# Ladme/groan_rs

Measured on AMD Instinct MI355X. Metric: frames/sec RMSD-fit, 1e6 atoms triclinic, 1/2/4/8 GPUs; HBM GB/s vs peak, higher is better.
Workload: dtype f32 (fp64 accumulators)

## Files before the change

groan_rs_amd/csrc/gr_api.hip:

```cpp
#include <hip/hip_runtime.h>

#include <cmath>
#include <cstdio>
#include <cstdlib>
#include <cstring>
#include <map>
#include <string>
#include <vector>

#include "../../include/groan_hip.h"
#include "gr_container.h"
#include "gr_kernels.h"
#include "gr_hot.h"
#include "gr_resident.h"
#include "gr_small.h"
#include "gr_xtc.h"
#include "gr_shape.h"
#include "gr_xtc_dev.h"
#include "gr_xtc_enc_dev.h"
#include "gr_trr.h"
#include "gr_cellgrid.h"
#include "gr_textio.h"
#include "gr_pool.h"
#include <set>
// ... 71 lines not shown
    int stream_wgs_cu = 0;
    int translate_rows = 1;
    int center_resident = 1;
    uint64_t cen_res_launches = 0, cen_res_redone = 0;
    int res_fit_last = 0;
    struct Metro { uint64_t shape = 0; double free_ns = 0, T_ns = 0, best_ns = 0, fail_ns = 0; uint32_t off_for = 0, held = 0; } metro;
    uint64_t res_metro_period_ns = 0, res_last_turn_ns = 0, res_late_permille = 0, res_sclk_mhz = 0;
    int wall_khz = 100000;
    uint32_t res_max_wgs = 0;
    int res_test_no_start = 0;
    uint32_t res_test_abort_at = 0xFFFFFFFFu;
    uint32_t res_skip = 0, res_backoff = 0;
    uint32_t *res_progress = nullptr;
    unsigned long long *res_wgrec = nullptr; size_t res_wgrec_cap = 0;
    unsigned long long *res_rec = nullptr;
    uint32_t *res_abort = nullptr;
    uint32_t *res_words_host = nullptr;
    struct ResOut { GrFrameState st[GR_MAX_BATCH]; uint32_t words[16]; alignas(64) uint32_t seq; };
    ResOut *res_out = nullptr, *res_out_dev = nullptr;
    uint32_t res_seq = 0;
    uint32_t res_checkin = 0, res_closed = 0;
    uint32_t res_late_seen[2] = { 0, 0 };
    uint64_t res_lean_segments = 0, res_sync_fallbacks = 0;
    GrShapeSet *shape_set_dev = nullptr;
    unsigned long long *shape_mask_dev = nullptr, *shape_mask_host = nullptr; size_t shape_mask_cap = 0;
    uint32_t res_epoch = 0;
    bool res_in_use = false;
    uint64_t res_launches = 0, res_handshake_misses = 0, res_aborts = 0, res_redone_frames = 0;
    GrFrameState *state_dev = nullptr;
    GrFrameState *state_host = nullptr;
    GrFrameState *small_state = nullptr, *small_state_dev = nullptr;
    uint32_t *small_flag = nullptr, *small_flag_dev = nullptr;
    uint32_t small_seq = 0;
    uint32_t small_max = GR_SMALL_MAX_DEFAULT;
    uint64_t small_calls = 0, small_sync_fallbacks = 0;
    uint32_t *bad_dev = nullptr;
// ... 388 lines not shown
            HIPCHK(c, hipStreamSynchronize(c->stream));
            if (w[0] != seq || w[words - 1] != seq) return fail(c, GR_E_HIP, "a single-wave kernel ended without publishing its result");
            break;
        }
    }
    std::atomic_thread_fence(std::memory_order_acquire);
    c->small_calls++;
    return GR_OK;
}

static int res_next_epoch(gr_ctx *c, uint32_t *epoch) {
    if (++c->res_epoch == 0u) {
        HIPCHK(c, hipStreamSynchronize(c->stream));
        if (c->res_wgrec) HIPCHK(c, hipMemset(c->res_wgrec, 0, c->res_wgrec_cap * sizeof(unsigned long long)));
        HIPCHK(c, hipMemset(c->res_rec, 0, (size_t)GR_MAX_BATCH * 16 * sizeof(unsigned long long)));
        HIPCHK(c, hipMemset(c->res_abort + 2, 0, 2 * sizeof(uint32_t)));
        c->res_epoch = 1u;
    }
    *epoch = c->res_epoch;
    return GR_OK;
}
static int res_test_no_start(gr_ctx *c, uint32_t epoch) {
    if (!c->res_test_no_start) return GR_OK;
    const unsigned long long two = 2ull | ((unsigned long long)epoch << 32);
    c->res_test_no_start = 0;
    HIPCHK(c, hipMemcpyAsync(c->res_abort + 2, &two, sizeof two, hipMemcpyHostToDevice, c->stream));
    HIPCHK(c, hipStreamSynchronize(c->stream));
    return GR_OK;
}
template <int MODE>
static int res_close(gr_ctx *c, uint32_t nb, const double *fit_partials, uint32_t nparts, double sum_w, uint32_t epoch, bool fresh, uint32_t *seq) {
    const uint32_t sq = c->res_seq + 1u;
    k_res_close<MODE><<<dim3(nb), dim3(64), 0, c->stream>>>(fit_partials, nparts, sum_w, c->state_dev, c->res_rec, epoch, fresh ? 1u : 0u, c->res_abort, c->res_closed + nb,
                                                        c->res_out_dev->st, c->res_out_dev->words, &c->res_out_dev->seq, sq);
    HIPCHK(c, hipGetLastError());
    c->res_seq = sq; c->res_closed += nb; *seq = sq;
    return GR_OK;
}
static int res_collect(gr_ctx *c, uint32_t seq, uint32_t nb, uint32_t epoch, bool *started) {
    volatile uint32_t *w = &c->res_out->seq;
    const auto t0 = std::chrono::steady_clock::now();
    for (uint32_t spins = 0; *w != seq; ++spins) {
        if ((spins & 1023u) == 1023u && std::chrono::steady_clock::now() - t0 > std::chrono::milliseconds(20)) {
            c->res_sync_fallbacks++;
            HIPCHK(c, hipStreamSynchronize(c->stream));
            if (*w != seq) return fail(c, GR_E_HIP, "the kernel behind the resident pass ended without publishing its results");
            break;
        }
    }
    std::atomic_thread_fence(std::memory_order_acquire);
    memcpy(c->state_host, c->res_out->st, (size_t)nb * sizeof(GrFrameState));
    memcpy(c->res_words_host, c->res_out->words, 12 * sizeof(uint32_t));
    for (int k = 0; k < 2; ++k) { const uint32_t v = c->res_words_host[8 + k]; c->res_words_host[8 + k] = v - c->res_late_seen[k]; c->res_late_seen[k] = v; }
    *started = c->res_words_host[2] == 1u && c->res_words_host[3] == epoch;
    if (!*started || c->res_words_host[0]) HIPCHK(c, hipStreamSynchronize(c->stream));
    return GR_OK;
}

int center_stage(gr_ctx *c, uint32_t first_slot, uint32_t nf, const GrSel &sel, int kind, int weighted,
                 int mass_first, int target, int only_status = 0) {
    if (small_ok(c, sel)) {
// ... 189 lines not shown
    (void)hipSetDevice(c->device);
    if (c->copy_stream) (void)hipStreamSynchronize(c->copy_stream);
    if (c->stream) (void)hipStreamSynchronize(c->stream);
    resident_done(c);
    whole_release(c);
    for (auto &kv : c->groups) { if (kv.second.idx_dev) (void)hipFree(kv.second.idx_dev); if (kv.second.mask_dev) (void)hipFree(kv.second.mask_dev); }
    if (c->frames) (void)hipFree(c->frames);
    if (c->aos_up) (void)hipFree(c->aos_up);
    if (c->aos_dl) (void)hipFree(c->aos_dl);
    if (c->masses) (void)hipFree(c->masses);
    if (c->boxes_dev) (void)hipFree(c->boxes_dev);
    if (c->boxes_host) (void)hipHostFree(c->boxes_host);
    if (c->cen_partials) (void)hipFree(c->cen_partials);
    if (c->acc_partials) (void)hipFree(c->acc_partials);
    if (c->fit_partials) (void)hipFree(c->fit_partials);
    if (c->fuse_cnt) (void)hipFree(c->fuse_cnt);
    if (c->res_abort) (void)hipFree(c->res_abort);
    if (c->res_words_host) (void)hipHostFree(c->res_words_host);
    if (c->res_out) (void)hipHostFree(c->res_out);
    if (c->shape_set_dev) (void)hipFree(c->shape_set_dev);
    if (c->shape_mask_dev) (void)hipFree(c->shape_mask_dev);
    if (c->shape_mask_host) (void)hipHostFree(c->shape_mask_host);
    if (c->res_wgrec) (void)hipFree(c->res_wgrec);
    if (c->res_rec) (void)hipFree(c->res_rec);
    if (c->res_progress) (void)hipFree(c->res_progress);
    if (c->state_dev) (void)hipFree(c->state_dev);
    if (c->state_host) (void)hipHostFree(c->state_host);
    if (c->small_state) (void)hipHostFree(c->small_state);
    if (c->bad_dev) (void)hipFree(c->bad_dev);
    if (c->bad_host) (void)hipHostFree(c->bad_host);
// ... 875 lines not shown
    }
    GrResCtl ctl;
    memset(&ctl, 0, sizeof ctl);
    { const int se = res_next_epoch(c, &ctl.epoch); if (se) return se; }
    ctl.wgrec = c->res_wgrec; ctl.rec = c->res_rec; ctl.abort = c->res_abort; ctl.progress = c->res_progress; ctl.n_stream = res_stream; ctl.n_fin = n_fin;
    ctl.checkin_target = c->res_checkin + res_stream + n_fin; ctl.fresh_states = fresh_states ? 1u : 0u;
    ctl.wgs_frame = wgs; ctl.streams = streams; ctl.groups_wg = gwg;
    ctl.team_waves = resident_team_waves(wgs, streams);
    ctl.patience_ticks = (unsigned long long)c->wall_khz * 3000ull; ctl.start_ticks = (unsigned long long)c->wall_khz * 200ull;
    ctl.test_abort_frame = c->res_test_abort_at; c->res_test_abort_at = 0xFFFFFFFFu;
    ctl.metro_t16 = c->res_metro_ns >= 100 ? (uint32_t)std::min<uint64_t>(0xFFFFFFFFull, (uint64_t)c->res_metro_ns * (uint64_t)c->wall_khz * 16ull / 1000000ull) : 0u;
    ctl.metro_lead = (uint32_t)((uint64_t)c->wall_khz * 2000ull / 1000000ull);
    ctl.cen_weighted = weighted ? 1u : 0u; ctl.cen_dim_mask = (uint32_t)dim_mask;
    float *frames = c->frames; size_t stride = c->frame_stride; uint32_t slot0 = s0, nfr = nb, natoms = (uint32_t)c->n;
    const float *masses = c->masses; GrSel sel_arg = csel; const GrBox *boxes = c->boxes_dev; GrPlanDev plan; memset(&plan, 0, sizeof plan);
    GrFrameState *states = c->state_dev; double *fparts = nullptr;
    void *args[] = { &frames, &stride, &slot0, &nfr, &natoms, &masses, &sel_arg, &boxes, &plan, &states, &fparts, &ctl };
    bool ubox = true;
    for (uint32_t f = 1; f < nb && ubox; ++f) ubox = memcmp(&c->boxes_host[s0 + f], &c->boxes_host[s0], sizeof(GrBox)) == 0;
    const bool fit_last = c->res_fit_last ? c->res_fit_last == 2 : (uint64_t)res_stream * 10u >= (uint64_t)c->res_max_wgs * 9u;
    { const int sn = res_test_no_start(c, ctl.epoch); if (sn) return sn; }
    if (hipLaunchKernel(resident_center_fn(ubox, fit_last), dim3(res_stream + n_fin), dim3(GrResShape::LANES), args, GrResShape::LDS_BYTES, S) != hipSuccess) {
        (void)hipGetLastError();
        c->res_max_wgs = 0;
        return GR_OK;
    }
    c->res_checkin += res_stream + n_fin;
    uint32_t seq = 0; bool started = false;
    { const int sc = res_close<1>(c, nb, nullptr, 0u, 1.0, ctl.epoch, fresh_states, &seq); if (sc) return sc; }
    { const int sc = res_collect(c, seq, nb, ctl.epoch, &started); if (sc) return sc; }
    c->res_last_streams = streams;
    if (!started) {
        c->res_handshake_misses++;
        c->res_backoff = c->res_backoff ? std::min<uint32_t>(c->res_backoff * 2u, 1024u) : 4u;
        c->res_skip = c->res_backoff;
        return GR_OK;
    }
    c->res_backoff = 0;
    c->cen_res_launches++;
    if (fresh_states) c->res_lean_segments++;
    ran = true;
#ifdef GR_EXP_STEPTIME
    if (getenv("GR_STEPTIME")) {
        unsigned long long st[32];
// ... 363 lines not shown
                HIPCHK(c, hipMalloc(&c->fit_partials, need * sizeof(double)));
                c->fit_partials_cap = need;
            }
        }
        const bool fused = (lite || fast) && c->fuse;
        q.fused = fused;
        hipStream_t S = c->stream;
        uint32_t res_streams = 1, res_gwg = GR_RES_GROUPS;
        const bool res_msk = fit && msk && c->two_pass && p->dev.w_is_mass != 0;
        uint32_t res_wgs = resident_wgs(c, lite || res_msk, nb, sel, &res_streams, &res_gwg);
        if (res_wgs && !resident_acquire(c->device)) res_wgs = 0;
        if (res_wgs) c->res_in_use = true;
        if (res_wgs) {
            const uint32_t res_stream = res_wgs * res_streams;
            const uint32_t n_fin = std::min<uint32_t>(res_streams > 8 ? GR_RES_MAX_FIN : 8, c->res_max_wgs - res_stream);
            if ((size_t)nb * res_wgs * GrResShape::WAVES > c->fit_partials_cap) {
                if (c->fit_partials) (void)hipFree(c->fit_partials);
                c->fit_partials = nullptr; c->fit_partials_cap = 0;
                HIPCHK(c, hipMalloc(&c->fit_partials, (size_t)nb * res_wgs * GrResShape::WAVES * sizeof(double)));
                c->fit_partials_cap = (size_t)nb * res_wgs * GrResShape::WAVES;
            }
            const size_t rec_words = (size_t)nb * ((res_wgs + GR_RES_REC_PAD - 1u) & ~(uint32_t)(GR_RES_REC_PAD - 1u)) * GR_RES_REC_WORDS;
            if (rec_words > c->res_wgrec_cap) {
                if (c->res_wgrec) (void)hipFree(c->res_wgrec);
                c->res_wgrec = nullptr; c->res_wgrec_cap = 0;
                HIPCHK(c, hipMalloc(&c->res_wgrec, rec_words * sizeof(unsigned long long)));
                HIPCHK(c, hipMemsetAsync(c->res_wgrec, 0, rec_words * sizeof(unsigned long long), S));
                c->res_wgrec_cap = rec_words;
            }
            GrResCtl ctl;
            st = res_next_epoch(c, &ctl.epoch); if (st) return st;
            ctl.wgrec = c->res_wgrec; ctl.rec = c->res_rec; ctl.abort = c->res_abort; ctl.progress = c->res_progress; ctl.n_stream = res_stream; ctl.n_fin = n_fin;
            ctl.checkin_target = c->res_checkin + res_stream + n_fin; ctl.fresh_states = states_unset ? 1u : 0u;
            ctl.wgs_frame = res_wgs; ctl.streams = res_streams; ctl.groups_wg = res_gwg;
            ctl.team_waves = resident_team_waves(res_wgs, res_streams);
// ... 22 lines not shown
                ctl.dbg = getenv("GR_STEPTIME") ? dbg_dev : nullptr;
                g_steptime_dbg = ctl.dbg;
            }
#endif
#ifdef GR_EXP_TIMELINE
            {
                static unsigned long long *tl_dev = nullptr; static size_t tl_cap = 0;
                if (nb > tl_cap) { if (tl_dev) (void)hipFree(tl_dev); tl_dev = nullptr; tl_cap = 0; if (hipMalloc(&tl_dev, (size_t)nb * 8 * sizeof(unsigned long long)) == hipSuccess) tl_cap = nb; }
                ctl.tl = getenv("GR_TIMELINE") ? tl_dev : nullptr;
                if (ctl.tl) HIPCHK(c, hipMemsetAsync(ctl.tl, 0, (size_t)nb * 8 * sizeof(unsigned long long), S));
                q.tl_dev = ctl.tl;
            }
#endif
            float *frames = c->frames; size_t stride = c->frame_stride; uint32_t slot0 = s0, nfr = nb, natoms = (uint32_t)c->n;
            const float *masses = c->masses; GrSel sel_arg = sel; const GrBox *boxes = c->boxes_dev; GrPlanDev plan = res_msk ? plan_span : p->dev;
            GrFrameState *states = c->state_dev; double *fparts = c->fit_partials;
            void *args[] = { &frames, &stride, &slot0, &nfr, &natoms, &masses, &sel_arg, &boxes, &plan, &states, &fparts, &ctl };
            bool ubox = true;
            for (uint32_t f = 1; f < nb && ubox; ++f) ubox = memcmp(&c->boxes_host[s0 + f], &c->boxes_host[s0], sizeof(GrBox)) == 0;
#ifdef GR_EXP_NO_UBOX
            ubox = false;
#endif
            const bool whole = sel.start == 0 && sel.n == c->n;
            const bool fit_last = c->res_fit_last ? c->res_fit_last == 2 : (uint64_t)res_stream * 10u >= (uint64_t)c->res_max_wgs * 9u;
            const void *fn = resident_fn(p->dev.w_is_mass != 0, ubox, whole, fit_last);
            const uint32_t lanes = GrResShape::LANES, lds = GrResShape::LDS_BYTES;
            st = res_test_no_start(c, ctl.epoch); if (st) return st;
            if (c->profile) EVREC(c, c->pev[0], true, S);
            const hipError_t le = hipLaunchKernel(fn, dim3(res_stream + n_fin), dim3(lanes), args, lds, S);
            if (le == hipSuccess) {
                if (c->profile) EVREC(c, c->pev[1], true, S);
                c->res_checkin += res_stream + n_fin;
                q.res_fresh = states_unset; q.res_epoch = ctl.epoch;
                states_unset = false;
                st = res_close<0>(c, nb, c->fit_partials, res_wgs * GrResShape::WAVES, p->dev.sw, ctl.epoch, q.res_fresh, &q.res_seq); if (st) return st;
                q.resident = true; q.res_stream = res_stream; q.res_streams = res_streams;
                q.rmsd_fast = false;
                c->res_last_streams = res_streams;
            } else {
                (void)hipGetLastError();
                c->res_max_wgs = 0;
                resident_done(c);
            }
        }
        if (!q.resident) { st = zero_states(); if (st) return st; }
        for (uint32_t g = 0; g < n_groups && !q.resident; ++g) {
            const uint32_t f0 = g * sb, nf = std::min<uint32_t>(sb, nb - f0), nch = batch_chunks(c, sel, nf), gx = fit_grid(c, nf);
            GrAccPartial *parts = c->acc_partials + (size_t)f0 * GR_MAX_CHUNKS;
            if (c->profile) EVREC(c, c->pev[6 * g], true, S);
            if (lite) k_sums_pk<false><<<dim3(nch, nf), dim3(GR_WG), 0, S>>>(c->frames, c->frame_stride, s0 + f0, c->masses, sel, c->boxes_dev, p->dev, parts,
// ... 1302 lines not shown
```

groan_rs_amd/csrc/gr_resident.h:

```cpp
#pragma once
#include <type_traits>
#include "gr_hot.h"

struct GrResShape {
    static constexpr int LANES = 512, WAVES = LANES / 64;
#ifndef GR_RES_K
#define GR_RES_K 6
#endif
    static constexpr int K = GR_RES_K;
    static constexpr int R = 8;
    static constexpr int PARK_F4 = K * 3 * LANES;
    static constexpr int WSUM_F = R * WAVES * 32;
#ifdef GR_EXP_TIMELINE
    static constexpr int TL_BYTES = 128 * 4 * 8;
#else
    static constexpr int TL_BYTES = 0;
#endif
    static constexpr int LDS_BYTES = PARK_F4 * 16 + WSUM_F * 4 + R * WAVES * 8 + 3 * R * 4 + 2 * WAVES * 4 + TL_BYTES;
    static constexpr int REC_PER_WAVE = 256 / WAVES, LANES_PER_REC = 64 / REC_PER_WAVE, WORDS_PER_LANE = 32 / LANES_PER_REC;
};
#ifndef GR_RES_SLEEP
#define GR_RES_SLEEP 2
#endif
#ifndef GR_RES_BAL
// ... 17 lines not shown
    unsigned long long *wgrec;
    unsigned long long *rec;
    uint32_t *abort;
    uint32_t *progress;
    uint32_t epoch, n_stream, n_fin;
    uint32_t checkin_target;
    uint32_t fresh_states;
    uint32_t wgs_frame, streams;
    uint32_t groups_wg;
    uint32_t team_waves;
    unsigned long long patience_ticks, start_ticks;
    uint32_t test_abort_frame;
    uint32_t metro_t16;
    uint32_t metro_lead;
    uint32_t cen_weighted, cen_dim_mask;
#ifdef GR_EXP_TIMELINE
    unsigned long long *tl;
#endif
#ifdef GR_EXP_STEPTIME
    unsigned long long *dbg;
#endif
};

template <typename T> __device__ __forceinline__ T gr_ld_agent(const T *p) { return __hip_atomic_load(p, __ATOMIC_RELAXED, __HIP_MEMORY_SCOPE_AGENT); }
__device__ __forceinline__ float gr_first_f(float v) { return __uint_as_float((uint32_t)__builtin_amdgcn_readfirstlane((int)__float_as_uint(v))); }
__device__ __forceinline__ float gr_lane_f(unsigned long long v, int l) { return __uint_as_float((uint32_t)__builtin_amdgcn_readlane((int)(uint32_t)v, l)); }
__device__ __forceinline__ void gr_lds_release() { __builtin_amdgcn_fence(__ATOMIC_RELEASE, "workgroup", "local"); }
__device__ __forceinline__ void gr_lds_acquire() { __builtin_amdgcn_fence(__ATOMIC_ACQUIRE, "workgroup", "local"); }

#ifndef GR_RES_STORE_AUX
#define GR_RES_STORE_AUX 18
#endif
__device__ __forceinline__ void gr_buf_store_stream(__amdgpu_buffer_rsrc_t r, uint32_t byte_off, const float4 &v) {
    gr_i4 t; t.x = __float_as_int(v.x); t.y = __float_as_int(v.y); t.z = __float_as_int(v.z); t.w = __float_as_int(v.w);
    __builtin_amdgcn_raw_buffer_store_b128(t, r, (int)byte_off, 0, GR_RES_STORE_AUX);
}

enum { GR_RG_IN0 = 1u, GR_RG_IN1 = 2u, GR_RG_IN2 = 4u, GR_RG_IN3 = 8u, GR_RG_ANY = 16u , GR_RG_FULL = 32u ,
       GR_RG_EX0 = 64u, GR_RG_EX1 = 128u, GR_RG_EX2 = 256u, GR_RG_EX3 = 512u , GR_RG_EXALL = 1024u };
struct GrResGroup {
    bool valid;
    uint32_t flags;
    uint32_t b;
// ... 65 lines not shown
        if (__builtin_amdgcn_ballot_w64((Gr.flags & GR_RG_FULL) == 0u) != 0ull) {
            s01.x = (Gr.flags & GR_RG_IN0) ? s01.x : 0.f; s01.y = (Gr.flags & GR_RG_IN1) ? s01.y : 0.f;
            s23.x = (Gr.flags & GR_RG_IN2) ? s23.x : 0.f; s23.y = (Gr.flags & GR_RG_IN3) ? s23.y : 0.f;
        }
        const gr_v2f part = gr_v2_fma(w23, s23, w01 * s01);
        rs += part.x + part.y;
    }
    n.x01 += gr_v2(cx); n.y01 += gr_v2(cy); n.z01 += gr_v2(cz); n.x23 += gr_v2(cx); n.y23 += gr_v2(cy); n.z23 += gr_v2(cz);
    gr_rows_pairs(n, o0, o1, o2);
}

template <bool WMASS, bool UBOX, bool V, bool FL, int MODE = 0>
__global__ __launch_bounds__(GrResShape::LANES) void k_fit_resident(
    float *__restrict__ frames, size_t frame_stride, uint32_t first_slot, uint32_t nframes, uint32_t n_atoms,
    const float *__restrict__ masses, GrSel sel, const GrBox *__restrict__ boxes, GrPlanDev plan,
    GrFrameState *state, double *__restrict__ fit_partials, GrResCtl ctl) {
    typedef GrResShape S;
    constexpr uint32_t LANES = S::LANES, WAVES = S::WAVES, K = S::K, R = S::R;
    extern __shared__ float4 smem[];
    const uint32_t tid = threadIdx.x, lane = tid & 63u, wave = tid >> 6;
    const uint32_t n_pad = (ctl.wgs_frame + GR_RES_REC_PAD - 1u) & ~(uint32_t)(GR_RES_REC_PAD - 1u);

    __shared__ unsigned long long metro_t0;
    {
        __shared__ uint32_t verdict;
        if (tid == 0) {
            unsigned long long *vw = reinterpret_cast<unsigned long long *>(ctl.abort + 2);
            const unsigned long long vtag = (unsigned long long)ctl.epoch << 32;
            auto decide = [&](uint32_t v) {
                unsigned long long cur = gr_ld_agent(vw);
                while ((uint32_t)(cur >> 32) != ctl.epoch &&
// ... 6 lines not shown
                asm volatile("s_waitcnt vmcnt(0)" ::: "memory");
                decide(1u);
            }
            unsigned long long vv;
            uint32_t polls = 0;
            const unsigned long long t0 = wall_clock64();
            while ((uint32_t)((vv = gr_ld_agent(vw)) >> 32) != ctl.epoch) {
                if (++polls > GR_RES_START_PATIENCE || ((polls & 255u) == 0 && wall_clock64() - t0 > ctl.start_ticks)) decide(2u);
                __builtin_amdgcn_s_sleep(16);
            }
            const uint32_t v = (uint32_t)vv;
            verdict = v;
            if (v == 1u) { __builtin_amdgcn_fence(__ATOMIC_ACQUIRE, "agent"); metro_t0 = gr_ld_agent(reinterpret_cast<const unsigned long long *>(ctl.abort + 4)); }
        }
        __syncthreads();
        if (verdict != 1u) return;
    }

    if (blockIdx.x >= ctl.n_stream) {
        constexpr uint32_t RPW = S::REC_PER_WAVE;
        const uint32_t TW = ctl.team_waves, NT = WAVES / TW, team = wave / TW, wt = wave % TW;
        double *wtot = reinterpret_cast<double *>(smem);
        uint32_t *gave_up = reinterpret_cast<uint32_t *>(wtot + 2u * WAVES * 32u);
        if (tid == 0) *gave_up = 0u;
        __syncthreads();
        const unsigned long long tagv = (unsigned long long)ctl.epoch << 32;
        for (uint32_t f0 = (blockIdx.x - ctl.n_stream) * NT; f0 < nframes; f0 += ctl.n_fin * NT) {
            const uint32_t f = f0 + team < nframes ? f0 + team : nframes - 1u;
            const bool live = f0 + team < nframes;
            const GrBox *bp = boxes + first_slot + f;
            GrBox lb;
            lb.ax = bp->ax; lb.by = bp->by; lb.cz = bp->cz; lb.bx = bp->bx; lb.cx = bp->cx; lb.cy = bp->cy;
            lb.bcx = bp->bcx; lb.bcy = bp->bcy; lb.bcz = bp->bcz; lb.r_ws = bp->r_ws; lb.ortho = bp->ortho;
            float g0x, g0y, g0z;
            gr_pos_load(frames + (size_t)(first_slot + f) * frame_stride, sel.start, g0x, g0y, g0z);
            const int pre_status = ctl.fresh_states ? 0 : state[f].status;
            const uint32_t rec0 = wt * RPW < n_pad ? wt * RPW : 0u, nrec = wt * RPW < n_pad ? min(RPW, n_pad - wt * RPW) : 0u;
            const unsigned long long *src = ctl.wgrec + ((size_t)f * n_pad + rec0) * GR_RES_REC_WORDS;
            const __amdgpu_buffer_rsrc_t rr = gr_buf_rsrc(src, nrec * GR_RES_REC_WORDS * 8u);
            const uint32_t w0 = (lane & 15u) * 2u, rbase = wt * RPW + (lane >> 4);
            gr_i4 q[8];
            uint32_t polls = 0;
// ... 32 lines not shown
#pragma unroll
            for (uint32_t off = 16u; off < 64u; off <<= 1) {
                const double o0 = __shfl_xor(a0, (int)off, 64), o1 = __shfl_xor(a1, (int)off, 64);
                a0 = mx0 ? fmax(a0, o0) : a0 + o0;
                a1 = mx1 ? fmax(a1, o1) : a1 + o1;
            }
            if (lane < 16u) { wtot[wave * 32u + w0] = a0; wtot[wave * 32u + w0 + 1u] = a1; }
            __syncthreads();
            if (wt == 0 && lane < 31u) {
                double a = wtot[wave * 32u + lane];
                const bool mx = lane >= 19u;
                for (uint32_t wv = 1; wv < TW; ++wv) { const double o = wtot[(wave + wv) * 32u + lane]; a = mx ? fmax(a, o) : a + o; }
                wtot[(WAVES + team) * 32u + lane] = a;
            }
            gr_wave_sync();
            if (wt == 0 && lane == 0 && live) {
#ifdef GR_EXP_TIMELINE
                if (ctl.tl) ctl.tl[(size_t)f * 8 + 2] = wall_clock64();
#endif
                GrFrameState st = {};
                if (ctl.fresh_states) st.err_index = GR_NOIDX; else st = state[f];
#ifdef GR_EXP_TIMELINE
                if (ctl.tl) { if (st.status > 1000000) ctl.tl[0] = 0; ctl.tl[(size_t)f * 8 + 3] = wall_clock64(); }
#endif
                const bool lost = *gave_up != 0u;
                const double *t = wtot + (WAVES + team) * 32u;
                if (lost) {
                    if (pre_status == 0) st.status = GR_ST_ABORTED;
                } else if (MODE == 1) {
                    if (pre_status == 0) {
// ... 32 lines not shown
                if (ctl.tl) { if (st.R[0] > 1.0e30f) ctl.tl[0] = 0; ctl.tl[(size_t)f * 8 + 4] = wall_clock64(); }
#endif
                unsigned long long *o = ctl.rec + (size_t)f * 16;
                gr_st_agent(o + 0, tagv | (uint32_t)st.status);
#pragma unroll
                for (int k = 0; k < 3; ++k) gr_st_agent(o + 1 + k, tagv | __float_as_uint(st.shift[k]));
#pragma unroll
                for (int k = 0; k < 9; ++k) gr_st_agent(o + 4 + k, tagv | __float_as_uint(st.R[k]));
                const double cvx = t[1] / t[0], cvy = t[2] / t[0], cvz = t[3] / t[0];
#pragma unroll
                for (int a = 0; a < 3; ++a) {
                    const float t0 = (float)(-((double)st.R[a] * cvx + (double)st.R[3 + a] * cvy + (double)st.R[6 + a] * cvz));
                    gr_st_agent(o + 13 + a, tagv | __float_as_uint(t0));
                }
                state[f] = st;
#ifdef GR_EXP_TIMELINE
                if (ctl.tl) ctl.tl[(size_t)f * 8 + 5] = wall_clock64();
#endif
            }
            __syncthreads();
        }
        return;
    }

    const uint32_t ngroups = ((n_atoms + 255u) >> 8) << 6;
    const uint32_t wg_all = blockIdx.x, stream = wg_all / ctl.wgs_frame, wg = wg_all % ctl.wgs_frame, base = wg * ctl.groups_wg;
    const uint32_t glimit = min(base + ctl.groups_wg, ngroups);
    const uint32_t n_turns = nframes > stream ? (nframes - stream + ctl.streams - 1u) / ctl.streams : 0u;
    auto kf = [&](uint32_t k) { return stream + k * ctl.streams; };
    if (base + wave * 64u >= glimit) {
        if (lane == 0) ctl.progress[wg_all * WAVES + wave] = GR_RES_IDLE_WAVE;
        if (MODE == 0 && fit_partials) for (uint32_t k = lane; k < n_turns; k += 64u) fit_partials[((size_t)kf(k) * ctl.wgs_frame + wg) * WAVES + wave] = 0.0;
        return;
    }
    const uint32_t n_waves = min(WAVES, (glimit - base) >> 6);
    float4 *park = smem;
    float *wsum = reinterpret_cast<float *>(smem + S::PARK_F4);
    double *fsum = reinterpret_cast<double *>(wsum + S::WSUM_F);
    uint32_t *cnt_s = reinterpret_cast<uint32_t *>(fsum + R * WAVES);
    uint32_t *prog = cnt_s + 3 * R, *simd_of = prog + WAVES;
#ifdef GR_EXP_TIMELINE
    unsigned long long *tls = reinterpret_cast<unsigned long long *>(simd_of + WAVES);
    const bool tl_wg = ctl.tl != nullptr && wg_all == 0u;
#endif
    if (tid < 3 * R) cnt_s[tid] = 0u;
    if (lane == 0) { prog[wave] = 0u; simd_of[wave] = (uint32_t)__builtin_amdgcn_s_getreg((1 << 11) | (4 << 6) | 4) ; }
    __syncthreads();
// ... 461 lines not shown
                if (GB.valid) gr_res_fit_group<WMASS>(GB, rb.r0, rb.r1, rb.r2, T, B, boxp, cx, cy, cz, ob.r0, ob.r1, ob.r2, rs);
            }
        }
        {
#ifdef GR_EXP_NOSTORE
            const __amdgpu_buffer_rsrc_t out = gr_buf_rsrc(frames + (size_t)(first_slot + kf(j)) * frame_stride, 0u);
#else
            const __amdgpu_buffer_rsrc_t out = gr_buf_rsrc(frames + (size_t)(first_slot + kf(j)) * frame_stride, status == 0 ? slot_bytes : 0u);
#endif
            gr_buf_store_stream(out, offA, oa.r0); gr_buf_store_stream(out, offA + 1024u, oa.r1); gr_buf_store_stream(out, offA + 2048u, oa.r2);
            gr_buf_store_stream(out, offB, ob.r0); gr_buf_store_stream(out, offB + 1024u, ob.r1); gr_buf_store_stream(out, offB + 2048u, ob.r2);
        }
        n_fitted = j + 1u;
        if (MODE == 1) return;
        const float wtot = gr_wave_allsum_f32(rs);
        if (lane == 0) fit_partials[((size_t)kf(j) * ctl.wgs_frame + wg) * WAVES + wave] = (double)wtot;
    };

    Landing L0, L1;
    L0.a.r0 = L0.a.r1 = L0.a.r2 = L0.b.r0 = L0.b.r1 = L0.b.r2 = zero4; L0.gx = L0.gy = L0.gz = 0.f;
    L1 = L0;
    Rows Q0, Q1, Q2, Q3, Q4, Q5;
    Q0.r0 = Q0.r1 = Q0.r2 = zero4; Q1 = Q0; Q2 = Q0; Q3 = Q0; Q4 = Q0; Q5 = Q0;
    unsigned long long rv = 0ull;
    gate(0);
    if (n_turns) request(0, L0);
    const uint32_t n_iter = n_turns + K;
    const GrBoxU B0 = gr_box_uniform(boxes + first_slot);
    auto lds_put = [&](uint32_t slot, const Rows &rw) { park[(slot * 3 + 0) * LANES + tid] = rw.r0; park[(slot * 3 + 1) * LANES + tid] = rw.r1; park[(slot * 3 + 2) * LANES + tid] = rw.r2; };
    auto lds_get = [&](uint32_t slot) { Rows rw; rw.r0 = park[(slot * 3 + 0) * LANES + tid]; rw.r1 = park[(slot * 3 + 1) * LANES + tid]; rw.r2 = park[(slot * 3 + 2) * LANES + tid]; return rw; };
    auto step_sums_first = [&](uint32_t i, Landing &cur, Landing &nxt) {
// ... 91 lines not shown
#endif
        if (clk_wave) {
            const unsigned long long dc = (unsigned long long)clock64() - clk_c0, dw = (unsigned long long)wall_clock64() - clk_w0;
            gr_st_agent(ctl.abort + 10, (uint32_t)(dc >> 8)); gr_st_agent(ctl.abort + 11, (uint32_t)(dw >> 8));
        }
    }
#ifdef GR_EXP_TIMELINE
    if (tl_wg && wave == 0 && !bail) {
        for (uint32_t t = (n_turns > 128u ? n_turns - 128u : 0u) + lane; t < n_turns; t += 64u) {
            const size_t f = kf(t);
            ctl.tl[f * 8 + 0] = tls[(t & 127u) * 4u + 0u];
            ctl.tl[f * 8 + 6] = tls[(t & 127u) * 4u + 1u] | (tls[(t & 127u) * 4u + 2u] << 48);
        }
    }
#endif
}

template <int MODE>
__global__ __launch_bounds__(64) void k_res_close(const double *__restrict__ fit_partials, uint32_t nparts, double sum_w, GrFrameState *state,
                                                  const unsigned long long *__restrict__ rec, uint32_t epoch, uint32_t fresh_states, uint32_t *ctl_words,
                                                  uint32_t done_target, GrFrameState *out_states, uint32_t *out_words, uint32_t *out_seq, uint32_t seq) {
    constexpr uint32_t NW = sizeof(GrFrameState) / 4u, W_RMSD = offsetof(GrFrameState, rmsd) / 4u, W_STATUS = offsetof(GrFrameState, status) / 4u;
    static_assert(sizeof(GrFrameState) % 4u == 0 && NW <= 64u, "a frame state is exported by one wave, a word per lane");
    const uint32_t frame = blockIdx.x, lane = threadIdx.x;
    uint32_t *sw = reinterpret_cast<uint32_t *>(state + frame);
    uint32_t w = 0u;
    if (fresh_states && (uint32_t)(gr_ld_agent(rec + (size_t)frame * 16u) >> 32) != epoch) {
        GrFrameState z = {};
        z.err_index = GR_NOIDX; z.status = GR_ST_ABORTED;
        if (lane < NW) { w = reinterpret_cast<const uint32_t *>(&z)[lane]; sw[lane] = w; }
    } else if (lane < NW) w = sw[lane];
    const int status = __shfl((int)w, (int)W_STATUS, 64);
    if (MODE == 0 && status == 0) {
        double s0 = 0.0, s1 = 0.0, s2 = 0.0, s3 = 0.0;
        const double *p = fit_partials + (size_t)frame * nparts;
        uint32_t k = lane;
        for (; k + 192 < nparts; k += 256) { s0 += p[k]; s1 += p[k + 64]; s2 += p[k + 128]; s3 += p[k + 192]; }
        for (; k < nparts; k += 64) s0 += p[k];
        const double s = gr_wave_sum((s0 + s1) + (s2 + s3));
        float r = 0.0f;
        if (lane == 0) { r = (float)sqrt(fmax(s, 0.0) / sum_w); state[frame].rmsd = r; }
        r = __shfl(r, 0, 64);
        if (lane == W_RMSD) w = __float_as_uint(r);
    }
    if (lane < NW) reinterpret_cast<uint32_t *>(out_states + frame)[lane] = w;
    __threadfence_system();
    uint32_t n = 0u;
    if (lane == 0) n = __hip_atomic_fetch_add(ctl_words + 12, 1u, __ATOMIC_ACQ_REL, __HIP_MEMORY_SCOPE_AGENT) + 1u;
    n = (uint32_t)__builtin_amdgcn_readfirstlane((int)n);
    if (n != done_target) return;
    if (lane < 12u) out_words[lane] = gr_ld_agent(ctl_words + lane);
    __threadfence_system();
    if (lane == 0) __hip_atomic_store(out_seq, seq, __ATOMIC_RELEASE, __HIP_MEMORY_SCOPE_SYSTEM);
}
```

Before: 141,200.

## Fold the resident close pass into the persistent fit kernel

Removes the separate k_res_close launch. Per-frame RMSD reduction and state export now happen inside the resident kernel: finisher waves poll epoch-tagged fit partials and close frames while they keep working, and the last exiting wave publishes the control words and sequence number. Fit partials become 64-bit words carrying the epoch in the high half and the f32 sum in the low half, so completeness can be checked without a second kernel. This saves a launch and a serialised tail pass. In exchange it adds polling, exit counters and more complex termination logic, which risks stalls or deadlock-like waits if the counters mismatch.

```diff
diff --git a/groan_rs_amd/csrc/gr_api.hip b/groan_rs_amd/csrc/gr_api.hip
--- a/groan_rs_amd/csrc/gr_api.hip
+++ b/groan_rs_amd/csrc/gr_api.hip
@@ -109,12 +109,13 @@
     uint32_t *res_progress = nullptr;
     unsigned long long *res_wgrec = nullptr; size_t res_wgrec_cap = 0;
     unsigned long long *res_rec = nullptr;
+    unsigned long long *res_fitw = nullptr; size_t res_fitw_cap = 0;
     uint32_t *res_abort = nullptr;
     uint32_t *res_words_host = nullptr;
     struct ResOut { GrFrameState st[GR_MAX_BATCH]; uint32_t words[16]; alignas(64) uint32_t seq; };
     ResOut *res_out = nullptr, *res_out_dev = nullptr;
     uint32_t res_seq = 0;
-    uint32_t res_checkin = 0, res_closed = 0;
+    uint32_t res_checkin = 0, res_exits = 0, res_stream_exits = 0;
     uint32_t res_late_seen[2] = { 0, 0 };
     uint64_t res_lean_segments = 0, res_sync_fallbacks = 0;
     GrShapeSet *shape_set_dev = nullptr;
@@ -533,6 +534,7 @@
         HIPCHK(c, hipStreamSynchronize(c->stream));
         if (c->res_wgrec) HIPCHK(c, hipMemset(c->res_wgrec, 0, c->res_wgrec_cap * sizeof(unsigned long long)));
         HIPCHK(c, hipMemset(c->res_rec, 0, (size_t)GR_MAX_BATCH * 16 * sizeof(unsigned long long)));
+        if (c->res_fitw) HIPCHK(c, hipMemset(c->res_fitw, 0, c->res_fitw_cap * sizeof(unsigned long long)));
         HIPCHK(c, hipMemset(c->res_abort + 2, 0, 2 * sizeof(uint32_t)));
         c->res_epoch = 1u;
     }
@@ -547,14 +549,16 @@
     HIPCHK(c, hipStreamSynchronize(c->stream));
     return GR_OK;
 }
-template <int MODE>
-static int res_close(gr_ctx *c, uint32_t nb, const double *fit_partials, uint32_t nparts, double sum_w, uint32_t epoch, bool fresh, uint32_t *seq) {
-    const uint32_t sq = c->res_seq + 1u;
-    k_res_close<MODE><<<dim3(nb), dim3(64), 0, c->stream>>>(fit_partials, nparts, sum_w, c->state_dev, c->res_rec, epoch, fresh ? 1u : 0u, c->res_abort, c->res_closed + nb,
-                                                        c->res_out_dev->st, c->res_out_dev->words, &c->res_out_dev->seq, sq);
-    HIPCHK(c, hipGetLastError());
-    c->res_seq = sq; c->res_closed += nb; *seq = sq;
-    return GR_OK;
+static void res_ending(const gr_ctx *c, uint32_t res_stream, uint32_t n_fin, GrResCtl &ctl) {
+    ctl.exit_target = c->res_exits + (res_stream + n_fin) * GrResShape::WAVES;
+    ctl.stream_exit_target = c->res_stream_exits + res_stream * GrResShape::WAVES;
+    ctl.out_states = c->res_out_dev->st; ctl.out_words = c->res_out_dev->words; ctl.out_seq = &c->res_out_dev->seq; ctl.seq = c->res_seq + 1u;
+}
+static uint32_t res_launched(gr_ctx *c, uint32_t res_stream, uint32_t n_fin) {
+    c->res_checkin += res_stream + n_fin;
+    c->res_exits += (res_stream + n_fin) * GrResShape::WAVES;
+    c->res_stream_exits += res_stream * GrResShape::WAVES;
+    return ++c->res_seq;
 }
 static int res_collect(gr_ctx *c, uint32_t seq, uint32_t nb, uint32_t epoch, bool *started) {
     volatile uint32_t *w = &c->res_out->seq;
@@ -563,7 +567,7 @@
         if ((spins & 1023u) == 1023u && std::chrono::steady_clock::now() - t0 > std::chrono::milliseconds(20)) {
             c->res_sync_fallbacks++;
             HIPCHK(c, hipStreamSynchronize(c->stream));
-            if (*w != seq) return fail(c, GR_E_HIP, "the kernel behind the resident pass ended without publishing its results");
+            if (*w != seq) return fail(c, GR_E_HIP, "the resident pass ended without publishing its results");
             break;
         }
     }
@@ -783,6 +787,7 @@
     if (c->cen_partials) (void)hipFree(c->cen_partials);
     if (c->acc_partials) (void)hipFree(c->acc_partials);
     if (c->fit_partials) (void)hipFree(c->fit_partials);
+    if (c->res_fitw) (void)hipFree(c->res_fitw);
     if (c->fuse_cnt) (void)hipFree(c->fuse_cnt);
     if (c->res_abort) (void)hipFree(c->res_abort);
     if (c->res_words_host) (void)hipHostFree(c->res_words_host);
@@ -1688,7 +1693,8 @@
     ctl.cen_weighted = weighted ? 1u : 0u; ctl.cen_dim_mask = (uint32_t)dim_mask;
     float *frames = c->frames; size_t stride = c->frame_stride; uint32_t slot0 = s0, nfr = nb, natoms = (uint32_t)c->n;
     const float *masses = c->masses; GrSel sel_arg = csel; const GrBox *boxes = c->boxes_dev; GrPlanDev plan; memset(&plan, 0, sizeof plan);
-    GrFrameState *states = c->state_dev; double *fparts = nullptr;
+    GrFrameState *states = c->state_dev; unsigned long long *fparts = nullptr;
+    res_ending(c, res_stream, n_fin, ctl);
     void *args[] = { &frames, &stride, &slot0, &nfr, &natoms, &masses, &sel_arg, &boxes, &plan, &states, &fparts, &ctl };
     bool ubox = true;
     for (uint32_t f = 1; f < nb && ubox; ++f) ubox = memcmp(&c->boxes_host[s0 + f], &c->boxes_host[s0], sizeof(GrBox)) == 0;
@@ -1699,9 +1705,8 @@
         c->res_max_wgs = 0;
         return GR_OK;
     }
-    c->res_checkin += res_stream + n_fin;
-    uint32_t seq = 0; bool started = false;
-    { const int sc = res_close<1>(c, nb, nullptr, 0u, 1.0, ctl.epoch, fresh_states, &seq); if (sc) return sc; }
+    const uint32_t seq = res_launched(c, res_stream, n_fin);
+    bool started = false;
     { const int sc = res_collect(c, seq, nb, ctl.epoch, &started); if (sc) return sc; }
     c->res_last_streams = streams;
     if (!started) {
@@ -2095,11 +2100,13 @@
         if (res_wgs) {
             const uint32_t res_stream = res_wgs * res_streams;
             const uint32_t n_fin = std::min<uint32_t>(res_streams > 8 ? GR_RES_MAX_FIN : 8, c->res_max_wgs - res_stream);
-            if ((size_t)nb * res_wgs * GrResShape::WAVES > c->fit_partials_cap) {
-                if (c->fit_partials) (void)hipFree(c->fit_partials);
-                c->fit_partials = nullptr; c->fit_partials_cap = 0;
-                HIPCHK(c, hipMalloc(&c->fit_partials, (size_t)nb * res_wgs * GrResShape::WAVES * sizeof(double)));
-                c->fit_partials_cap = (size_t)nb * res_wgs * GrResShape::WAVES;
+            const size_t fit_words = (size_t)nb * res_wgs * GrResShape::WAVES;
+            if (fit_words > c->res_fitw_cap) {
+                if (c->res_fitw) (void)hipFree(c->res_fitw);
+                c->res_fitw = nullptr; c->res_fitw_cap = 0;
+                HIPCHK(c, hipMalloc(&c->res_fitw, fit_words * sizeof(unsigned long long)));
+                HIPCHK(c, hipMemsetAsync(c->res_fitw, 0, fit_words * sizeof(unsigned long long), S));
+                c->res_fitw_cap = fit_words;
             }
             const size_t rec_words = (size_t)nb * ((res_wgs + GR_RES_REC_PAD - 1u) & ~(uint32_t)(GR_RES_REC_PAD - 1u)) * GR_RES_REC_WORDS;
             if (rec_words > c->res_wgrec_cap) {
@@ -2152,7 +2159,8 @@
 #endif
             float *frames = c->frames; size_t stride = c->frame_stride; uint32_t slot0 = s0, nfr = nb, natoms = (uint32_t)c->n;
             const float *masses = c->masses; GrSel sel_arg = sel; const GrBox *boxes = c->boxes_dev; GrPlanDev plan = res_msk ? plan_span : p->dev;
-            GrFrameState *states = c->state_dev; double *fparts = c->fit_partials;
+            GrFrameState *states = c->state_dev; unsigned long long *fparts = c->res_fitw;
+            res_ending(c, res_stream, n_fin, ctl);
             void *args[] = { &frames, &stride, &slot0, &nfr, &natoms, &masses, &sel_arg, &boxes, &plan, &states, &fparts, &ctl };
             bool ubox = true;
             for (uint32_t f = 1; f < nb && ubox; ++f) ubox = memcmp(&c->boxes_host[s0 + f], &c->boxes_host[s0], sizeof(GrBox)) == 0;
@@ -2168,10 +2176,9 @@
             const hipError_t le = hipLaunchKernel(fn, dim3(res_stream + n_fin), dim3(lanes), args, lds, S);
             if (le == hipSuccess) {
                 if (c->profile) EVREC(c, c->pev[1], true, S);
-                c->res_checkin += res_stream + n_fin;
                 q.res_fresh = states_unset; q.res_epoch = ctl.epoch;
                 states_unset = false;
-                st = res_close<0>(c, nb, c->fit_partials, res_wgs * GrResShape::WAVES, p->dev.sw, ctl.epoch, q.res_fresh, &q.res_seq); if (st) return st;
+                q.res_seq = res_launched(c, res_stream, n_fin);
                 q.resident = true; q.res_stream = res_stream; q.res_streams = res_streams;
                 q.rmsd_fast = false;
                 c->res_last_streams = res_streams;
diff --git a/groan_rs_amd/csrc/gr_resident.h b/groan_rs_amd/csrc/gr_resident.h
--- a/groan_rs_amd/csrc/gr_resident.h
+++ b/groan_rs_amd/csrc/gr_resident.h
@@ -55,6 +55,10 @@
     uint32_t metro_t16;
     uint32_t metro_lead;
     uint32_t cen_weighted, cen_dim_mask;
+    uint32_t exit_target, stream_exit_target;
+    GrFrameState *out_states;
+    uint32_t *out_words;
+    uint32_t *out_seq, seq;
 #ifdef GR_EXP_TIMELINE
     unsigned long long *tl;
 #endif
@@ -68,6 +72,21 @@
 __device__ __forceinline__ float gr_lane_f(unsigned long long v, int l) { return __uint_as_float((uint32_t)__builtin_amdgcn_readlane((int)(uint32_t)v, l)); }
 __device__ __forceinline__ void gr_lds_release() { __builtin_amdgcn_fence(__ATOMIC_RELEASE, "workgroup", "local"); }
 __device__ __forceinline__ void gr_lds_acquire() { __builtin_amdgcn_fence(__ATOMIC_ACQUIRE, "workgroup", "local"); }
+
+__device__ __forceinline__ void gr_res_leave(const GrResCtl &ctl, uint32_t lane, uint32_t weight, bool streaming) {
+    uint32_t last = 0u;
+    if (lane == 0) {
+        if (streaming) (void)__hip_atomic_fetch_add(ctl.abort + 13, weight, __ATOMIC_RELEASE, __HIP_MEMORY_SCOPE_AGENT);
+        last = __hip_atomic_fetch_add(ctl.abort + 12, weight, __ATOMIC_ACQ_REL, __HIP_MEMORY_SCOPE_AGENT) + weight == ctl.exit_target ? 1u : 0u;
+    }
+    if (__builtin_amdgcn_readfirstlane((int)last) == 0) return;
+    if (lane < 12u) ctl.out_words[lane] = gr_ld_agent(ctl.abort + lane);
+    __threadfence_system();
+    if (lane == 0) __hip_atomic_store(ctl.out_seq, ctl.seq, __ATOMIC_RELEASE, __HIP_MEMORY_SCOPE_SYSTEM);
+}
+__device__ __forceinline__ void gr_res_export(const GrResCtl &ctl, uint32_t f, uint32_t lane, uint32_t w) {
+    if (lane < sizeof(GrFrameState) / 4u) __hip_atomic_store(reinterpret_cast<uint32_t *>(ctl.out_states + f) + lane, w, __ATOMIC_RELAXED, __HIP_MEMORY_SCOPE_SYSTEM);
+}
 
 #ifndef GR_RES_STORE_AUX
 #define GR_RES_STORE_AUX 18
@@ -163,7 +182,7 @@
 __global__ __launch_bounds__(GrResShape::LANES) void k_fit_resident(
     float *__restrict__ frames, size_t frame_stride, uint32_t first_slot, uint32_t nframes, uint32_t n_atoms,
     const float *__restrict__ masses, GrSel sel, const GrBox *__restrict__ boxes, GrPlanDev plan,
-    GrFrameState *state, double *__restrict__ fit_partials, GrResCtl ctl) {
+    GrFrameState *state, unsigned long long *__restrict__ fit_words, GrResCtl ctl) {
     typedef GrResShape S;
     constexpr uint32_t LANES = S::LANES, WAVES = S::WAVES, K = S::K, R = S::R;
     extern __shared__ float4 smem[];
@@ -200,7 +219,33 @@
             if (v == 1u) { __builtin_amdgcn_fence(__ATOMIC_ACQUIRE, "agent"); metro_t0 = gr_ld_agent(reinterpret_cast<const unsigned long long *>(ctl.abort + 4)); }
         }
         __syncthreads();
-        if (verdict != 1u) return;
+        if (verdict != 1u) {
+            __shared__ uint32_t last_out;
+            if (tid == 0) {
+                if (blockIdx.x < ctl.n_stream) (void)__hip_atomic_fetch_add(ctl.abort + 13, WAVES, __ATOMIC_RELAXED, __HIP_MEMORY_SCOPE_AGENT);
+                last_out = __hip_atomic_fetch_add(ctl.abort + 12, WAVES, __ATOMIC_ACQ_REL, __HIP_MEMORY_SCOPE_AGENT) + WAVES == ctl.exit_target ? 1u : 0u;
+            }
+            __syncthreads();
+            if (last_out == 0u) return;
+            constexpr uint32_t NW = sizeof(GrFrameState) / 4u, W_STATUS = offsetof(GrFrameState, status) / 4u, W_ERR = offsetof(GrFrameState, err_index) / 4u;
+            for (uint32_t f = wave; f < nframes; f += WAVES) {
+                uint32_t *sw = reinterpret_cast<uint32_t *>(state + f);
+                uint32_t w = 0u;
+                if (ctl.fresh_states) {
+                    w = lane == W_STATUS ? (uint32_t)GR_ST_ABORTED : (lane == W_ERR ? GR_NOIDX : 0u);
+                    if (lane < NW) sw[lane] = w;
+                } else if (lane < NW) w = gr_ld_agent(sw + lane);
+                gr_res_export(ctl, f, lane, w);
+            }
+            __syncthreads();
+            if (wave == 0) {
+                __threadfence_system();
+                if (lane < 12u) ctl.out_words[lane] = gr_ld_agent(ctl.abort + lane);
+                __threadfence_system();
+                if (lane == 0) __hip_atomic_store(ctl.out_seq, ctl.seq, __ATOMIC_RELEASE, __HIP_MEMORY_SCOPE_SYSTEM);
+            }
+            return;
+        }
     }
 
     if (blockIdx.x >= ctl.n_stream) {
@@ -211,7 +256,59 @@
         if (tid == 0) *gave_up = 0u;
         __syncthreads();
         const unsigned long long tagv = (unsigned long long)ctl.epoch << 32;
-        for (uint32_t f0 = (blockIdx.x - ctl.n_stream) * NT; f0 < nframes; f0 += ctl.n_fin * NT) {
+        const bool closer = MODE == 0 && wt == (TW > 1u ? 1u : 0u);
+        const uint32_t first_f = (blockIdx.x - ctl.n_stream) * NT + team, round_step = ctl.n_fin * NT;
+        uint32_t c_round = 0u, rnd = 0u;
+        const uint32_t nparts = ctl.wgs_frame * WAVES;
+        auto close_frame = [&](uint32_t fc, bool block) -> bool {
+            constexpr uint32_t NW = sizeof(GrFrameState) / 4u, W_RMSD = offsetof(GrFrameState, rmsd) / 4u, W_STATUS = offsetof(GrFrameState, status) / 4u;
+            static_assert(sizeof(GrFrameState) % 4u == 0 && NW <= 64u, "a frame state is exported by one wave, a word per lane");
+            uint32_t *sw = reinterpret_cast<uint32_t *>(state + fc);
+            uint32_t w = lane < NW ? gr_ld_agent(sw + lane) : 0u;
+            if (__builtin_amdgcn_readlane((int)w, (int)W_STATUS) == 0) {
+                const unsigned long long *p = fit_words + (size_t)fc * nparts;
+                uint32_t polls = 0;
+                bool final_look = false, complete = false;
+                const unsigned long long t0 = wall_clock64();
+                double s = 0.0;
+                for (;;) {
+                    double s0 = 0.0, s1 = 0.0, s2 = 0.0, s3 = 0.0;
+                    bool ok = true;
+                    uint32_t k = lane;
+                    for (; k + 192u < nparts; k += 256u) {
+                        const unsigned long long a = gr_ld_agent(p + k), b = gr_ld_agent(p + k + 64u), c2 = gr_ld_agent(p + k + 128u), d = gr_ld_agent(p + k + 192u);
+                        ok = ok && (uint32_t)(a >> 32) == ctl.epoch && (uint32_t)(b >> 32) == ctl.epoch && (uint32_t)(c2 >> 32) == ctl.epoch && (uint32_t)(d >> 32) == ctl.epoch;
+                        s0 += (double)__uint_as_float((uint32_t)a); s1 += (double)__uint_as_float((uint32_t)b);
+                        s2 += (double)__uint_as_float((uint32_t)c2); s3 += (double)__uint_as_float((uint32_t)d);
+                    }
+                    for (; k < nparts; k += 64u) {
+                        const unsigned long long a = gr_ld_agent(p + k);
+                        ok = ok && (uint32_t)(a >> 32) == ctl.epoch;
+                        s0 += (double)__uint_as_float((uint32_t)a);
+                    }
+                    s = (s0 + s1) + (s2 + s3);
+                    if (__builtin_amdgcn_ballot_w64(!ok) == 0ull) { complete = true; break; }
+                    if (!block) return false;
+                    if (final_look) break;
+                    if (gr_ld_agent(ctl.abort + 13) == ctl.stream_exit_target) { __builtin_amdgcn_fence(__ATOMIC_ACQUIRE, "agent"); final_look = true; continue; }
+                    if (++polls > GR_RES_PATIENCE || ((polls & 255u) == 0 && wall_clock64() - t0 > ctl.patience_ticks)) {
+                        if (lane == 0) gr_st_agent(ctl.abort, 1u);
+                        break;
+                    }
+                    __builtin_amdgcn_s_sleep(8);
+                }
+                if (complete) {
+                    s = gr_wave_sum(s);
+                    float r = 0.0f;
+                    if (lane == 0) { r = (float)sqrt(fmax(s, 0.0) / plan.sw); state[fc].rmsd = r; }
+                    r = gr_first_f(r);
+                    if (lane == W_RMSD) w = __float_as_uint(r);
+                }
+            }
+            gr_res_export(ctl, fc, lane, w);
+            return true;
+        };
+        for (uint32_t f0 = (blockIdx.x - ctl.n_stream) * NT; f0 < nframes; f0 += ctl.n_fin * NT, ++rnd) {
             const uint32_t f = f0 + team < nframes ? f0 + team : nframes - 1u;
             const bool live = f0 + team < nframes;
             const GrBox *bp = boxes + first_slot + f;
@@ -274,6 +371,12 @@
                 wtot[(WAVES + team) * 32u + lane] = a;
             }
             gr_wave_sync();
+            auto look = [&]() {
+                if (!closer || c_round >= rnd) return;
+                const uint32_t fc = first_f + c_round * round_step;
+                if (f / ctl.streams >= fc / ctl.streams + K + 1u && close_frame(fc, false)) ++c_round;
+            };
+            if (TW > 1u) look();
             if (wt == 0 && lane == 0 && live) {
 #ifdef GR_EXP_TIMELINE
                 if (ctl.tl) ctl.tl[(size_t)f * 8 + 2] = wall_clock64();
@@ -336,12 +439,26 @@
                     gr_st_agent(o + 13 + a, tagv | __float_as_uint(t0));
                 }
                 state[f] = st;
+                if (MODE == 1) {
+                    uint32_t sw[sizeof(GrFrameState) / 4u];
+                    __builtin_memcpy(sw, &st, sizeof st);
+#pragma unroll
+                    for (uint32_t k = 0; k < sizeof(GrFrameState) / 4u; ++k) __hip_atomic_store(reinterpret_cast<uint32_t *>(ctl.out_states + f) + k, sw[k], __ATOMIC_RELAXED, __HIP_MEMORY_SCOPE_SYSTEM);
+                }
 #ifdef GR_EXP_TIMELINE
                 if (ctl.tl) ctl.tl[(size_t)f * 8 + 5] = wall_clock64();
 #endif
             }
+            if (TW == 1u) look();
             __syncthreads();
         }
+        if (closer)
+            for (; c_round < rnd; ++c_round) {
+                const uint32_t fc = first_f + c_round * round_step;
+                if (fc < nframes) (void)close_frame(fc, true);
+            }
+        __syncthreads();
+        if (wave == 0) { __threadfence_system(); gr_res_leave(ctl, lane, WAVES, false); }
         return;
     }
 
@@ -352,7 +469,8 @@
     auto kf = [&](uint32_t k) { return stream + k * ctl.streams; };
     if (base + wave * 64u >= glimit) {
         if (lane == 0) ctl.progress[wg_all * WAVES + wave] = GR_RES_IDLE_WAVE;
-        if (MODE == 0 && fit_partials) for (uint32_t k = lane; k < n_turns; k += 64u) fit_partials[((size_t)kf(k) * ctl.wgs_frame + wg) * WAVES + wave] = 0.0;
+        if (MODE == 0 && fit_words) for (uint32_t k = lane; k < n_turns; k += 64u) gr_st_agent(fit_words + ((size_t)kf(k) * ctl.wgs_frame + wg) * WAVES + wave, (unsigned long long)ctl.epoch << 32);
+        gr_res_leave(ctl, lane, 1u, true);
         return;
     }
     const uint32_t n_waves = min(WAVES, (glimit - base) >> 6);
@@ -844,7 +962,7 @@
         n_fitted = j + 1u;
         if (MODE == 1) return;
         const float wtot = gr_wave_allsum_f32(rs);
-        if (lane == 0) fit_partials[((size_t)kf(j) * ctl.wgs_frame + wg) * WAVES + wave] = (double)wtot;
+        if (lane == 0) gr_st_agent(fit_words + ((size_t)kf(j) * ctl.wgs_frame + wg) * WAVES + wave, ((unsigned long long)ctl.epoch << 32) | __float_as_uint(wtot));
     };
 
     Landing L0, L1;
@@ -966,42 +1084,5 @@
         }
     }
 #endif
+    gr_res_leave(ctl, lane, 1u, true);
 }
-
-template <int MODE>
-__global__ __launch_bounds__(64) void k_res_close(const double *__restrict__ fit_partials, uint32_t nparts, double sum_w, GrFrameState *state,
-                                                  const unsigned long long *__restrict__ rec, uint32_t epoch, uint32_t fresh_states, uint32_t *ctl_words,
-                                                  uint32_t done_target, GrFrameState *out_states, uint32_t *out_words, uint32_t *out_seq, uint32_t seq) {
-    constexpr uint32_t NW = sizeof(GrFrameState) / 4u, W_RMSD = offsetof(GrFrameState, rmsd) / 4u, W_STATUS = offsetof(GrFrameState, status) / 4u;
-    static_assert(sizeof(GrFrameState) % 4u == 0 && NW <= 64u, "a frame state is exported by one wave, a word per lane");
-    const uint32_t frame = blockIdx.x, lane = threadIdx.x;
-    uint32_t *sw = reinterpret_cast<uint32_t *>(state + frame);
-    uint32_t w = 0u;
-    if (fresh_states && (uint32_t)(gr_ld_agent(rec + (size_t)frame * 16u) >> 32) != epoch) {
-        GrFrameState z = {};
-        z.err_index = GR_NOIDX; z.status = GR_ST_ABORTED;
-        if (lane < NW) { w = reinterpret_cast<const uint32_t *>(&z)[lane]; sw[lane] = w; }
-    } else if (lane < NW) w = sw[lane];
-    const int status = __shfl((int)w, (int)W_STATUS, 64);
-    if (MODE == 0 && status == 0) {
-        double s0 = 0.0, s1 = 0.0, s2 = 0.0, s3 = 0.0;
-        const double *p = fit_partials + (size_t)frame * nparts;
-        uint32_t k = lane;
-        for (; k + 192 < nparts; k += 256) { s0 += p[k]; s1 += p[k + 64]; s2 += p[k + 128]; s3 += p[k + 192]; }
-        for (; k < nparts; k += 64) s0 += p[k];
-        const double s = gr_wave_sum((s0 + s1) + (s2 + s3));
-        float r = 0.0f;
-        if (lane == 0) { r = (float)sqrt(fmax(s, 0.0) / sum_w); state[frame].rmsd = r; }
-        r = __shfl(r, 0, 64);
-        if (lane == W_RMSD) w = __float_as_uint(r);
-    }
-    if (lane < NW) reinterpret_cast<uint32_t *>(out_states + frame)[lane] = w;
-    __threadfence_system();
-    uint32_t n = 0u;
-    if (lane == 0) n = __hip_atomic_fetch_add(ctl_words + 12, 1u, __ATOMIC_ACQ_REL, __HIP_MEMORY_SCOPE_AGENT) + 1u;
-    n = (uint32_t)__builtin_amdgcn_readfirstlane((int)n);
-    if (n != done_target) return;
-    if (lane < 12u) out_words[lane] = gr_ld_agent(ctl_words + lane);
-    __threadfence_system();
-    if (lane == 0) __hip_atomic_store(out_seq, seq, __ATOMIC_RELEASE, __HIP_MEMORY_SCOPE_SYSTEM);
-}
```

Result: slower. 104,500 (-26.0%).
